# Happy-ZZX/PL-VIWO

Hardware: AMD Instinct MI355X
Metric: frames/sec (track+EKF update), 752x480 mono, 250 pts+80 lines; ATE vs CPU ref (higher is better)
Workload: dtype f64

## Files before the change

pl-viwo_amd/csrc/jacobian_api.hip:

```cpp
#include <algorithm>
#include <vector>

#include <chrono>
#include "jacobian_kernels.hpp"
#include "nullspace_core.hpp"
#include "update_kernels.hpp"
#include "update_state.hpp"
#include "camera_tracks.hpp"

using namespace plv;

#define TRY(expr)                  \
  do {                             \
    int _rc = (expr);              \
    if (_rc != PLV_OK) return _rc; \
  } while (0)

namespace {

int check_views(const plv_state_view *st, const plv_tracks *tr) {
  if (!st || !tr || st->n_clones < 1 || !st->clone_time || !st->clone_R || !st->clone_p || !st->clone_R_fej ||
      !st->clone_p_fej || !st->clone_state_id || tr->n_feat < 1 || !tr->obs_ptr || !tr->obs_time || !tr->obs_uv ||
      !tr->p_FinG || !tr->p_FinG_fej) {
    set_last_error("jacobians: null view field");
// ... 380 lines not shown
  us->pt_tri_p = (const double *)(us->tri.as<char>() + ft.o_p), us->pt_tri_ok = (const unsigned char *)(us->tri.as<char>() + ft.o_ok), us->pt_tri_F = F;
  const bool mirrored = ctx->mirror2_taken;
  ctx->mirror2_src = nullptr, ctx->mirror2_dst = nullptr, ctx->mirror2_bytes = 0, ctx->mirror2_taken = false;
  if (!mirrored)
    PLV_HIP_CHECK(plv::memcpy_async(us->h_tri.p, us->tri.as<char>() + ft.o_p, mirror_bytes, hipMemcpyDeviceToHost, ctx->stream));
  ph_b.stop();
  plv::frame_mark("@ point chain enqueued");
  if (J.chain_events) (void)hipEventRecord(g_ce[2], ctx->stream);
  J.pending = true, J.mirrored = mirrored, J.rc = rc, J.F = F, J.spec = spec != nullptr, J.max_sel = max_sel;
  J.o_p = ft.o_p, J.o_member = ft.o_member, J.o_words = ft.o_words;
  return PLV_OK;
}

int plv_points_update_collect(plv_ctx *ctx, double *p_out, uint8_t *ok_out, double *err_out, uint8_t *accepted, int *n_rows, double *dx,
                              void (*before_wait)(void *), void *before_wait_arg, uint8_t *member, int *spec_count, int *spec_over) {
  if (!ctx || !p_out || !ok_out || !err_out || !accepted || !dx) return PLV_E_BADARG;
  auto *us = plv_update_state(ctx);
  PointJob &J = point_job(ctx);
  if (!J.pending) {
    set_last_error("plv_points_update_collect: no point update was submitted");
    return PLV_E_BADARG;
  }
  J.pending = false;
  int rc = J.rc;
  const int F = J.F;
  plv::HostPhase ph_c("points fused: host work inside the wait");
  if (before_wait) before_wait(before_wait_arg);
  if (rc == PLV_OK && ctx->wait_poll && us->done_ev) {
    while (hipEventQuery(us->done_ev) == hipErrorNotReady || plv::knob(plv::PLV_KNOB_CHAIN_ALWAYS)) {
      if (ctx->wait_poll(ctx->wait_poll_arg)) break;
      for (int i = 0; i < 32; ++i) __builtin_ia32_pause();
    }
  }
  ph_c.stop();
  plv::frame_mark("@ host work inside the point wait done");
  plv::NsScope ns_pw(plv::counters().points_wait_ns);
  plv::HostPhase ph_d("points fused: wait");
  if (J.spec && us->spec_save_seq) spec_save_arm(ctx, us, true);
  if (rc == PLV_OK) rc = plv_msckf_update_resident_wait(ctx, accepted, n_rows, dx);
  spec_save_arm(ctx, us, false);
  if (rc != PLV_OK || !J.mirrored) PLV_HIP_CHECK(plv::stream_sync(ctx->stream));
  ph_d.stop();
  plv::frame_mark("@ point update collected");
  if (J.chain_events) {
    const double host_us = std::chrono::duration<double, std::micro>(std::chrono::steady_clock::now() - J.t_entry).count();
    (void)hipEventSynchronize(g_ce[2]);
    float a = 0.f, b = 0.f;
    if (hipEventElapsedTime(&a, g_ce[0], g_ce[1]) == hipSuccess && hipEventElapsedTime(&b, g_ce[1], g_ce[2]) == hipSuccess) {
      plv::host_phases().add("points fused: DEVICE entry -> Jacobian launch done", a * 1e3);
      plv::host_phases().add("points fused: DEVICE Jacobian done -> last kernel done", b * 1e3);
      plv::host_phases().add("points fused: HOST entry -> results read", host_us);
    }
  }
  const char *h = us->h_tri.as<char>();
  memcpy(p_out, h, (size_t)F * 24);
  memcpy(err_out, h + (size_t)F * 24, (size_t)F * 8);
  memcpy(ok_out, h + (size_t)F * 32, (size_t)F);
  if (J.spec) {
    if (member) memcpy(member, h + (J.o_member - J.o_p), (size_t)F);
    const int *w = (const int *)(h + (J.o_words - J.o_p));
    if (spec_count) *spec_count = w[0];
    if (spec_over) *spec_over = w[1] ? 1 : ((w[3] && w[4] >= J.max_sel) ? 2 : 0);
  } else {
    if (spec_count) *spec_count = 0;
    if (spec_over) *spec_over = 0;
  }
// ... 587 lines not shown
```

pl-viwo_amd/csrc/line_api.hip:

```cpp
#include <algorithm>
#include <chrono>
#include <cmath>
#include <cstring>
#include <atomic>
#include <condition_variable>
#include <functional>
#include <memory>
#include <map>
#include <mutex>
#include <thread>
#include <unordered_map>
#include <vector>

#include "line_host.hpp"
#include "cam_models.hpp"
#include "line_kernels.hpp"
#include "update_state.hpp"
#include "plv_internal.hpp"
#include "camera_tracks.hpp"

using namespace plv;
using namespace plv::linehost;

int plv_tracker_last(plv_ctx *ctx, float *pts, uint64_t *ids, int cap, int *n);
// ... 65 lines not shown
  int early_w = 0, early_h = 0;
  int pending_which = -1, pending_fed = -1;
  bool defer_finish = false;
  std::function<void()> deferred;
  std::atomic<int> defer_state{0};
  struct TriState {
    bool valid = false;
    plv_state_view view;
    std::vector<double> clone_time, clone_R, clone_p;
    std::vector<int> clone_id;
  } tri_state;
  std::vector<float> cached;
  int cached_which = -1, cached_fed = -1;
  std::mutex mtx;
  linehost::Job job;
  std::thread worker;
  std::mutex jm;
  std::condition_variable jcv;
  std::atomic<int> job_state{0};
  struct FeedJob {
    plv_ctx *ctx = nullptr;
    double timestamp = 0, vps[6] = {0, 0, 0, 0, 0, 0};
    double K8[8] = {0, 0, 0, 0, 0, 0, 0, 0};
    int cam_model = 0;
    std::vector<float> pts;
    std::vector<uint64_t> pids;
    int rc = PLV_OK;
    bool pool_on = false;
    PoolArgs pool_args;
  } feed;
  std::atomic<int> feed_state{0};
  std::chrono::steady_clock::time_point job_posted, feed_posted;
  linehost::HostStage host;
};

std::mutex g_mtx;
std::unordered_map<plv_ctx *, LineTracker *> g_lt;
LineTracker *ltr(plv_ctx *ctx, bool run_deferred = true);


void form_line_pool(LineTracker *T, const PoolArgs &A, LinePool &R);
void discard_line_pool(LineTracker *T);
int (*g_feed_impl)(plv_ctx *, LineTracker *, double, const double *, int, const float *, const uint64_t *, const double *, int) = nullptr;
void line_worker(LineTracker *T) {
  for (;;) {
    bool do_detect = false, do_feed = false, do_deferred = false;
    {
      std::unique_lock<std::mutex> lk(T->jm);
      wait_polling(lk, T->jcv, [&] { return T->job_state == 1 || T->job_state == -1 || T->feed_state == 1 || T->defer_state == 1; });
      if (T->job_state == -1) return;
      do_deferred = T->defer_state == 1;
      do_detect = !do_deferred && T->job_state == 1;
      do_feed = !do_deferred && !do_detect && T->feed_state == 1;
    }
    if (do_deferred) {
      std::function<void()> f;
      f.swap(T->deferred);
      if (f) f();
      {
        std::lock_guard<std::mutex> lk(T->jm);
        T->defer_state = 2;
      }
      T->jcv.notify_all();
      continue;
    }
    if (do_feed) {
      LineTracker::FeedJob &F = T->feed;
      if (plv::host_phases().on)
        plv::host_phases().add("line worker: feed job starts after its post", std::chrono::duration<double, std::micro>(std::chrono::steady_clock::now() - T->feed_posted).count());
      const auto Fs = std::chrono::steady_clock::now();
      plv::counters().w_feed_start_ns += (unsigned long long)std::chrono::duration_cast<std::chrono::nanoseconds>(Fs - T->feed_posted).count();
      const int rc = g_feed_impl(F.ctx, T, F.timestamp, F.vps, (int)F.pids.size(), F.pts.data(), F.pids.data(), F.K8, F.cam_model);
      if (rc == PLV_OK && F.pool_on) {
        discard_line_pool(T);
        form_line_pool(T, F.pool_args, T->pool_prep);
      }
      F.pool_on = false;
      plv::frame_mark("@ (worker) line feed + pool done");
      plv::counters().w_feed_ns += (unsigned long long)std::chrono::duration_cast<std::chrono::nanoseconds>(std::chrono::steady_clock::now() - Fs).count();
      {
        std::lock_guard<std::mutex> lk(T->jm);
        F.rc = rc;
        T->feed_state = 2;
      }
      T->jcv.notify_all();
      continue;
    }
    const bool timing = plv::knob(plv::PLV_KNOB_LINE_TIMING);
    auto W0 = std::chrono::steady_clock::now();
    (void)hipSetDevice(T->job.device);
    int rc = PLV_OK;
    if (plv::event_sync(T->edges_ready) != hipSuccess) rc = PLV_E_DEVICE;
    if (rc == PLV_OK && T->job.hlab && plv::event_sync(T->labels_ready) != hipSuccess) rc = PLV_E_DEVICE;
    auto W1 = std::chrono::steady_clock::now();
    if (rc == PLV_OK) rc = host_extract(&T->host, T->job, timing);
    {
      auto ns = [](auto a, auto b) { return (unsigned long long)std::chrono::duration_cast<std::chrono::nanoseconds>(b - a).count(); };
      plv::counters().w_wake_ns += ns(T->job_posted, W0);
      plv::counters().w_maps_ns += ns(W0, W1);
      plv::counters().w_extract_ns += ns(W1, std::chrono::steady_clock::now());
    }
    if (plv::host_phases().on)
      plv::host_phases().add("line worker: detect job, post to done", std::chrono::duration<double, std::micro>(std::chrono::steady_clock::now() - T->job_posted).count());
    plv::frame_mark("@ (worker) line detection done");
    if (timing) {
      auto W2 = std::chrono::steady_clock::now();
      auto us = [](auto a, auto b) { return std::chrono::duration<double, std::micro>(b - a).count(); };
      fprintf(stderr, "line worker: woke %.1f us after the post, edge maps %.1f us, walk + fit %.1f us\n", us(T->job_posted, W0), us(W0, W1), us(W1, W2));
    }
    {
      std::lock_guard<std::mutex> lk(T->jm);
      T->job.rc = rc;
      if (T->job_state == 1) T->job_state = 2;
    }
    T->jcv.notify_all();
  }
}
// ... 815 lines not shown
  bool any = false;
  for (int l = 0; l < Lp; ++l) any = (J.flags[l] = J.valid_n[l] >= 2) || any;
  if (!any) {
    J.stage = LinesJob::FUSED_NOTHING;
    return PLV_OK;
  }
  plv::HostPhase ph_cols("update_lines: columns");
  int rc = plv_line_jacobian_columns(st, &all, J.cols.data(), (int)J.cols.size(), &J.k);
  ph_cols.stop();
  if (rc == PLV_OK && J.k > 0) {
    plv::HostPhase ph_sub("update_lines: fused submit (gate prepare + stage + upload + launch)");
    ctx->gate_rows_hint = 2 * J.most_valid;
    ch.on = chained;
    rc = plv_lines_update_fused_submit(ctx, st, st_tri, &all, J.flags.data(), cap, J.k, J.cols.data(), 2 * opt->max_obs, st->sigma_pix * st->sigma_pix,
                                       opt->chi2_mult);
    ch.on = false;
    if (rc == PLV_OK) {
      J.stage = LinesJob::FUSED_LAUNCHED;
      return PLV_OK;
    }
  }
  if (rc == PLV_OK) {
    J.stage = LinesJob::FUSED_NOTHING;
    return PLV_OK;
  }
  J.stage = LinesJob::FAILED, J.rc = rc;
  return PLV_OK;
}

}
namespace plv {
int plv_camera_lines_submit_chained(plv_ctx *ctx, const plv_state_view *st, const plv_update_options *opt, int cap) {
  if (!ctx || !st || !opt || opt->cpi || st->n_clones < 2 || opt->max_obs < 2 || st->dt_state_id >= 0 || !ctx->chain.ready) return 0;
  LineTracker *T = ltr(ctx);
  if (T->ujob.pending || T->feed.rc != PLV_OK) return 0;
  plv::frame_mark("@ chained first half starts");
  plv::HostPhase ph("update_lines: first half inside the point update's wait (chained)");
  T->tri_state.valid = false;
  (void)lines_first_half(ctx, T, st, st, opt, cap, T->ujob, true);
  if (T->ujob.stage == LinesJob::TWO_STEP) {
    T->pool_prep = std::move(T->ujob.LP);
    T->pool_prep.valid = true;
    T->ujob = LinesJob();
    return 0;
  }
  T->ujob.pending = true;
  plv::frame_mark("@ chained first half done (line launch enqueued)");
  if (T->ujob.stage == LinesJob::FUSED_LAUNCHED) ++plv::counters().chained;
  return 1;
}

int plv_camera_lines_job_pending(plv_ctx *ctx) { return ltr(ctx, false)->ujob.pending ? 1 : 0; }
void plv_camera_lines_job_abort2(plv_ctx *ctx, int keep_pool) {
  LineTracker *T = ltr(ctx, false);
  if (!T->ujob.pending) return;
  (void)plv::stream_sync(ctx->stream);
  ctx->gate_stage.on = 0, ctx->gate_stage_taken = false;
  T->pool_prep = std::move(T->ujob.LP);
  T->pool_prep.valid = true;
  if (!keep_pool) discard_line_pool(T);
  T->ujob = LinesJob();
}
void plv_camera_lines_job_abort(plv_ctx *ctx) { plv_camera_lines_job_abort2(ctx, 0); }
}
extern "C" {

int plv_camera_update_lines(plv_ctx *ctx, const plv_state_view *st, const plv_update_options *opt, double *dx,
                            plv_update_result *res, uint64_t *line_ids, uint8_t *accepted_out, double *lines_out, int cap) {
  if (!ctx || !st || !opt || !dx || !res || st->n_clones < 2 || opt->max_obs < 2) return PLV_E_BADARG;
  LineTracker *T = ltr(ctx);
  *res = plv_update_result{0, 0, 0, 0, 0, PLV_OK, 0, 0, 0};
  const bool timing = plv::knob(plv::PLV_KNOB_UPDATE_TIMING);
  plv::NsScope ns_lines(plv::counters().lines_ns);
  plv::HostPhase ph_all("update_lines: whole call");
  plv::RoctxRange rx_line("[Time-Cam] LINE update");
  auto since = [&](std::chrono::steady_clock::time_point a) { return std::chrono::duration<double, std::micro>(std::chrono::steady_clock::now() - a).count(); };
  LinesJob Jlocal;
  const bool resumed = T->ujob.pending && T->ujob.cap == cap && T->ujob.n_clones == st->n_clones && T->ujob.state_time == opt->state_time &&
                       T->ujob.t_prev_frame == opt->t_prev_frame;
  if (T->ujob.pending && !resumed) {
    plv::set_last_error("plv_camera_update_lines: a chained submission for another window is pending");
    return PLV_E_BADARG;
// ... 231 lines not shown
```

pl-viwo_amd/csrc/plv_ctx.hpp:

```cpp
#pragma once
#include <hip/hip_runtime.h>
#include <sys/resource.h>

#include "gate_stage.hpp"
#include <cstdint>
#include <cstdio>
#include <execinfo.h>
#include <cstring>
#include <algorithm>
#include <atomic>
#include <chrono>
#include <cstdlib>
#include <mutex>
#include <string>
#include <unordered_map>
#include <vector>

#include "../../include/plviwo.h"

namespace plv {

void set_last_error(const char *fmt, ...);

#define PLV_HIP_CHECK(expr)                                                              \
// ... 408 lines not shown
    bool ready = false, on = false;
    std::vector<double> q;
    std::vector<int> ids;
    double qe[4] = {0, 0, 0, 1};
    std::vector<int> anc_ptr, anc_f;
    std::vector<unsigned char> anc_has_old;
    std::vector<double> anc_old;
  } chain;
  int *applied_word = nullptr;
  bool applied_used = false;
  const int *cap_words = nullptr;
  int cap = 0;
  double *cov_save = nullptr;
  unsigned *cov_save_word = nullptr;
  unsigned cov_save_seq = 0;
  const int *skip_word = nullptr;
  const void *mirror2_src = nullptr;
  void *mirror2_dst = nullptr;
  size_t mirror2_bytes = 0;
  bool mirror2_taken = false;
  bool probe = false, probe_done = false;
  const void *probe_src = nullptr;
  void *probe_dst = nullptr;
  int probe_stride_a = 0, probe_off_b = 0, probe_stride_b = 0;
  void (*probe_hook)(void *) = nullptr;
  void *probe_hook_arg = nullptr;

  plv::GateStage gate_stage{};
  bool gate_stage_taken = false;
  int gate_rows_hint = 0;

  int (*wait_poll)(void *) = nullptr;
  void *wait_poll_arg = nullptr;

  void *fe_state = nullptr;
};
```

pl-viwo_amd/csrc/plv_internal.hpp:

```cpp
#pragma once
#include <cstdint>

#include "../../include/plviwo.h"

struct plv_ctx_update_state;

struct plv_points_spec {
  int n_flow;
  const int *li;
  const uint8_t *meta, *prevalid;
  const float *d_flow_p1, *d_flow_n1;
  const uint8_t *d_flow_mask;
};

namespace plv {

plv_ctx_update_state *plv_update_state(plv_ctx *ctx);
int plv_update_gate_prepare(plv_ctx *ctx, int F, int fdim, int k, int ld, double sigma2, double chi2_mult, double res_norm_gate, int probe);
int plv_prior_prefetch(plv_ctx *ctx, int phase, const int *d_cols, int k, int F, int mp_max);

int plv_state_vars_check(int n_var, const plv_state_var *vars, int n_dx);

void plv_frontend_destroy(plv_ctx *ctx);
int plv_feed_image_enqueue(plv_ctx *ctx, const uint8_t *img, int stride);
int plv_front_fed_count(plv_ctx *ctx);
int plv_front_match_device(plv_ctx *ctx, const float **d_p1, const float **d_n1, const uint8_t **d_mask, int *n);
const uint8_t *plv_front_level0(plv_ctx *ctx, int which, int *w, int *h);
int plv_front_quiesce(plv_ctx *ctx);
int plv_perform_detection_ahead(plv_ctx *ctx, const uint8_t *mask, const float *pts, const uint64_t *ids, int n_in);

void plv_tracker_destroy(plv_ctx *ctx);
int plv_point_chain_lookup(plv_ctx *ctx, uint64_t id);
int plv_point_used_lookup(plv_ctx *ctx, uint64_t id, double *p);
void plv_point_anchor_fill(plv_ctx *ctx, int Lp, const int *pt_ptr, const int *pt_ids, int chained, double *anchor, uint8_t *has);
void plv_point_used_cleanup(plv_ctx *ctx, double t_oldest);
void plv_tracker_run_deferred(void *ctx);

void plv_line_tracker_destroy(plv_ctx *ctx);
int plv_line_prefetch_enabled(plv_ctx *ctx);
void plv_line_edges_early(plv_ctx *ctx, const uint8_t *d_raw, int W, int H, const unsigned *d_hist);
int plv_line_tracker_feed_async_points(plv_ctx *ctx, double timestamp, const double *vps, int np, const float *pts, const uint64_t *pids);
void plv_line_defer_finish(plv_ctx *ctx, int on);
void plv_line_run_deferred(plv_ctx *ctx);
int plv_line_pool_prepare(plv_ctx *ctx, const plv_state_view *st, const plv_update_options *opt);
void plv_line_feed_pool_args(plv_ctx *ctx, const plv_state_view *st, const plv_update_options *opt);
void plv_line_pool_discard(plv_ctx *ctx);
int plv_line_db_size_after_feed(plv_ctx *ctx);
int plv_camera_lines_submit_chained(plv_ctx *ctx, const plv_state_view *st, const plv_update_options *opt, int cap);
int plv_camera_lines_job_pending(plv_ctx *ctx);
void plv_camera_lines_job_abort2(plv_ctx *ctx, int keep_pool);
void plv_camera_lines_job_abort(plv_ctx *ctx);

int plv_points_update_submit(plv_ctx *ctx, const plv_state_view *st, const plv_tracks *all, const plv_tri_options *tri,
                             const uint8_t *flags, int max_sel, int k, const int *col_to_state, int ld, double sigma2,
                             double chi2_mult, double res_norm_gate, const plv_points_spec *spec);
int plv_points_update_collect(plv_ctx *ctx, double *p_out, uint8_t *ok_out, double *err_out, uint8_t *accepted, int *n_rows, double *dx,
                              void (*before_wait)(void *), void *before_wait_arg, uint8_t *member, int *spec_count, int *spec_over);
int plv_points_spec_undo(plv_ctx *ctx);
int plv_points_update_fused(plv_ctx *ctx, const plv_state_view *st, const plv_tracks *all, const plv_tri_options *tri,
                            const uint8_t *flags, int max_sel, int k, const int *col_to_state, int ld, double sigma2,
                            double chi2_mult, double res_norm_gate, double *p_out, uint8_t *ok_out, double *err_out,
                            uint8_t *accepted, int *n_rows, double *dx, void (*before_wait)(void *), void *before_wait_arg);
int plv_lines_update_fused(plv_ctx *ctx, const plv_state_view *st, const plv_state_view *st_tri, const plv_line_tracks *all,
                           const uint8_t *flags, int max_sel, int k, const int *col_to_state, int ld, double sigma2,
                           double chi2_mult, double *lines_out, uint8_t *ok_out, uint8_t *accepted, int *n_rows, double *dx,
                           void (*before_wait)(void *), void *before_wait_arg);
int plv_lines_update_fused_submit(plv_ctx *ctx, const plv_state_view *st, const plv_state_view *st_tri, const plv_line_tracks *all,
                                  const uint8_t *flags, int max_sel, int k, const int *col_to_state, int ld, double sigma2, double chi2_mult);
int plv_lines_update_fused_finish(plv_ctx *ctx, double sigma2, double chi2_mult, double *lines_out, uint8_t *ok_out, uint8_t *accepted,
                                  int *n_rows, double *dx, void (*before_wait)(void *), void *before_wait_arg);

}
// ... 1 lines not shown
```

pl-viwo_amd/csrc/tracker_api.hip:

```cpp
#include <algorithm>
#include <functional>
#include <memory>
#include <mutex>
#include <unordered_map>
#include <vector>

#include <sys/resource.h>
#include "plv_ctx.hpp"
#include "update_state.hpp"
#include "plv_internal.hpp"
#include "gate_stage.hpp"
#include "camera_tracks.hpp"

using plv::Track;

namespace {

struct Tracker {
  std::vector<float> pts_last;
  std::vector<uint64_t> ids_last;
  std::vector<uint8_t> mask_last;
  uint64_t currid = 0;
  int detect_ahead = 2;
  bool ahead_deferred = false;
  bool defer_db = false;
  const plv_state_view *early_st = nullptr;
  const plv_update_options *early_lines = nullptr;
  int early_cap = 0;
  std::unordered_map<uint64_t, int> chain_index;
  bool chain_ok = false;
  std::function<void()> deferred_db;
  std::unordered_map<uint64_t, Track> db;
  struct UsedPoint {
    double p[3], newest;
  };
  std::unordered_map<uint64_t, UsedPoint> used;
  struct Listed {
    uint64_t id;
    Track tr;
    double p[3];
  };
  std::vector<Listed> last_slam, last_init;
  std::vector<uint64_t> dec_ids;
  std::vector<double> dec_vals;
  const plv_state_view *spec_st = nullptr;
  const plv_update_options *spec_opt = nullptr;
  std::function<void(int, const float *, const uint64_t *)> points_ready;
  unsigned long long feed_seq = 0;
  std::vector<double> frame_t;
  struct Spec {
    bool active = false;
    double t_prev_frame = 0, state_time = 0, dt = 0, t_oldest = 0, t_oldest2 = 0;
    int n_clones = 0, max_msckf = 0, max_obs = 0, k = 0, F = 0;
    std::unordered_map<uint64_t, int> index;
    std::vector<uint64_t> ids;
    std::vector<int> ptr, li, cols;
    std::vector<uint8_t> meta, prevalid, flags;
    std::vector<double> ot;
    std::vector<float> ouv, ouvn;
  } spec;
  std::mutex mtx;
};

std::mutex g_mtx;
std::unordered_map<plv_ctx *, Tracker *> g_trk;
Tracker *trk(plv_ctx *ctx) {
  std::lock_guard<std::mutex> lk(g_mtx);
  auto it = g_trk.find(ctx);
  if (it != g_trk.end()) return it->second;
// ... 331 lines not shown
    Track &tr = tp[i] ? *tp[i] : T->db[ids[i]];
    if (tr.t.capacity() == 0) {
      tr.t.reserve(32);
      tr.uv.reserve(64);
      tr.uvn.reserve(64);
    }
    tr.t.push_back(timestamp);
    tr.uv.push_back(x);
    tr.uv.push_back(y);
    tr.uvn.push_back(n1[2 * i]);
    tr.uvn.push_back(n1[2 * i + 1]);
  }
  T->pts_last.swap(good);
  T->ids_last.swap(good_ids);
  keep_mask();
  T->ahead_deferred = T->detect_ahead == 2 && !T->ids_last.empty();
  if (T->detect_ahead == 1 && !T->ids_last.empty())
    (void)plv_perform_detection_ahead(ctx, mask, T->pts_last.data(), T->ids_last.data(), (int)T->ids_last.size());
  return PLV_OK;
}

static void start_detection_ahead(void *arg) {
  plv_ctx *ctx = (plv_ctx *)arg;
  Tracker *T = trk(ctx);
  {
    std::lock_guard<std::mutex> lk(T->mtx);
    if (T->ahead_deferred) {
      T->ahead_deferred = false;
      (void)plv_perform_detection_ahead(ctx, T->mask_last.empty() ? nullptr : T->mask_last.data(), T->pts_last.data(), T->ids_last.data(),
                                        (int)T->ids_last.size());
    }
  }
}
static int poll_line_pool(void *arg) {
  plv_ctx *ctx = (plv_ctx *)arg;
  Tracker *T = trk(ctx);
  if (!T->early_lines || !T->early_st) return 1;
  if (!plv_line_pool_prepare(ctx, T->early_st, T->early_lines)) return 0;
  if (plv::host_phases().on) {
    plv::host_phases().add("chain: pool ready inside the point wait (count)", 1.0);
    if (!T->chain_ok) plv::host_phases().add("chain: no - the point pool exceeds max_msckf or holds no candidate (count)", 1.0);
    if (!ctx->chain.ready) plv::host_phases().add("chain: no - state variables not chainable (count)", 1.0);
    if (!plv_update_state(ctx)->applied_armed) plv::host_phases().add("chain: no - the point launch did not arm the applied word (count)", 1.0);
  }
  if (T->chain_ok && ctx->chain.ready && plv_update_state(ctx)->applied_armed && !plv::knob(plv::PLV_KNOB_NO_CHAIN))
    (void)plv_camera_lines_submit_chained(ctx, T->early_st, T->early_lines, T->early_cap);
  return 1;
}
}
namespace plv {
int plv_point_chain_lookup(plv_ctx *ctx, uint64_t id) {
  Tracker *T = trk(ctx);
  auto it = T->chain_index.find(id);
  return it == T->chain_index.end() ? -1 : it->second;
}
}
extern "C" {

int plv_decision_trace(plv_ctx *ctx, int on) {
  if (!ctx) return PLV_E_BADARG;
  ctx->decision_trace = on != 0;
  return PLV_OK;
}
int plv_last_point_decisions(plv_ctx *ctx, uint64_t *ids, double *vals, int cap, int *n) {
  if (!ctx || !n || cap < 0 || (cap > 0 && (!ids || !vals))) return PLV_E_BADARG;
  Tracker *T = trk(ctx);
  *n = (int)T->dec_ids.size();
  if (*n > cap) return cap == 0 ? PLV_OK : PLV_E_CAPACITY;
  std::copy(T->dec_ids.begin(), T->dec_ids.end(), ids);
  std::copy(T->dec_vals.begin(), T->dec_vals.end(), vals);
  return PLV_OK;
}

int plv_tracker_detect_ahead(plv_ctx *ctx, int on) {
  if (!ctx) return PLV_E_BADARG;
  Tracker *T = trk(ctx);
  std::lock_guard<std::mutex> lk(T->mtx);
  T->detect_ahead = on < 0 ? 0 : on > 2 ? 2 : on;
  return PLV_OK;
}
// ... 261 lines not shown
    if (!spec_done) std::fill(dx, dx + ctx->cov_n, 0.0);
    return finish(PLV_OK);
  }
  std::vector<double> pf(3 * (size_t)Fp), err(Fp);
  std::vector<uint8_t> ok(Fp);
  plv_tracks all{};
  all.n_feat = Fp;
  all.obs_ptr = ptr.data();
  all.obs_time = ot.data();
  all.obs_uv = ouv.data();
  all.obs_uvn = ouvn.data();
  if (cpi.on) {
    all.res_R = cpi.R.data();
    all.res_p = cpi.p.data();
  }
  std::vector<int> cols(ctx->cfg.max_state_dim > 0 ? ctx->cfg.max_state_dim : 1024);
  int k = 0, n_rows = 0, rc = PLV_OK;
  const bool fused = !opt->cpi && opt->max_slam == 0 && most_valid <= opt->max_obs;
  ph_pool.stop();
  rx_get.stop();
  plv::frame_mark("@ update_points: pool + staging done");
  plv::RoctxRange rx_upd("[Time-Cam] MSCKF update");
  plv::HostPhase ph_dev("update_points: device submission + wait");
  std::vector<uint8_t> acc_all(Fp, 0);
  bool fused_ran = false;
  if (fused && spec_done) {
    std::copy(s_pf.begin(), s_pf.end(), pf.begin());
    std::copy(s_err.begin(), s_err.end(), err.begin());
    std::copy(s_ok.begin(), s_ok.end(), ok.begin());
    std::copy(s_acc.begin(), s_acc.end(), acc_all.begin());
    n_rows = s_rows;
    res->status = s_status;
    fused_ran = true;
  } else if (fused) {
    std::vector<uint8_t> flags(Fp);
    bool any = false;
    for (int f = 0; f < Fp; ++f) any = (flags[f] = valid_n[f] >= 2) || any;
    if (any) {
      all.p_FinG = all.p_FinG_fej = pf.data();
      rc = plv_jacobian_columns(st, &all, cols.data(), (int)cols.size(), &k);
      if (rc == PLV_OK && k > 0) {
        ctx->gate_rows_hint = 2 * most_valid;
        T->chain_index.clear();
        T->chain_ok = Fp <= opt->max_msckf;
        if (T->chain_ok && T->early_lines)
          for (int f = 0; f < Fp; ++f)
            if (flags[f]) T->chain_index.emplace(pool[f].id, f);
        plv::frame_mark("@ update_points: columns done, fused call");
        rc = plv_points_update_fused(ctx, st, &all, &opt->tri, flags.data(), opt->max_msckf, k, cols.data(), 2 * opt->max_obs,
                                     st->sigma_pix * st->sigma_pix, opt->chi2_mult, 3.0, pf.data(), ok.data(), err.data(), acc_all.data(),
                                     &n_rows, dx, start_detection_ahead, ctx);
        T->chain_ok = false;
        res->status = rc == PLV_E_NOT_PSD ? rc : PLV_OK;
        if (rc == PLV_E_NOT_PSD) {
          rc = PLV_OK;
          std::fill(dx, dx + ctx->cov_n, 0.0);
        }
        fused_ran = rc == PLV_OK;
      }
      if (rc != PLV_OK) {
        for (Cand &c : pool) give_back_all(unused, c);
        return finish(rc);
      }
    }
  } else {
    start_detection_ahead(ctx);
    rc = plv_triangulate(ctx, st, &all, &opt->tri, pf.data(), ok.data(), err.data());
    if (rc != PLV_OK) {
      for (Cand &c : pool) give_back_all(unused, c);
      return finish(rc);
    }
  }
  ph_dev.stop();
  rx_upd.stop();
  if (ctx->decision_trace) {
    const double nan = std::numeric_limits<double>::quiet_NaN();
    T->dec_ids.resize(Fp);
    T->dec_vals.assign((size_t)Fp * PLV_DECISION_VALUES, nan);
    std::vector<double> tri(4 * (size_t)Fp, nan), gate(3 * (size_t)Fp, nan);
    if (fused_ran && ctx->dec_F == Fp) {
      PLV_HIP_CHECK(hipMemcpy(tri.data(), ctx->d_tri_dbg.p, tri.size() * 8, hipMemcpyDeviceToHost));
      if (ctx->dec_gate) PLV_HIP_CHECK(hipMemcpy(gate.data(), ctx->d_gate_dec.p, gate.size() * 8, hipMemcpyDeviceToHost));
    }
    ctx->dec_F = 0, ctx->dec_gate = false;
    for (int f = 0; f < Fp; ++f) {
      double *v = &T->dec_vals[(size_t)f * PLV_DECISION_VALUES];
      T->dec_ids[f] = pool[f].id;
      v[0] = valid_n[f], v[1] = ok[f], v[2] = ok[f] ? err[f] : nan, v[3] = fused_ran ? acc_all[f] : nan;
      for (int i = 0; i < 4; ++i) v[4 + i] = tri[4 * (size_t)f + i];
      for (int i = 0; i < 3; ++i) v[8 + i] = gate[3 * (size_t)f + i];
    }
  }
  plv::RoctxRange rx_db("[Time-Cam] DB clan up");
  plv::HostPhase ph_post("update_points: selection + database");
  std::vector<int> sel;
  std::vector<int> n_skip(Fp, 0);
  for (int f = 0; f < Fp; ++f) {
    Cand &c = pool[f];
    if ((int)sel.size() >= opt->max_msckf) {
      give_back_all(unused, c);
      continue;
    }
    const int valid = valid_n[f];
    if (valid >= 2 && ok[f]) {
      std::lock_guard<std::mutex> lk(T->mtx);
      Tracker::UsedPoint &u = T->used[c.id];
      std::copy(pf.begin() + 3 * (size_t)f, pf.begin() + 3 * (size_t)f + 3, u.p);
      u.newest = c.tr.t.back();
    }
    if (valid < 2 || !ok[f] || !(err[f] < 3.0)) {
      give_back_all(unused, c);
      continue;
    }
    if (valid >= opt->init_min_meas && opt->n_slam + (int)T->last_init.size() < opt->max_slam) {
      Tracker::Listed e{c.id, Track{}, {pf[3 * (size_t)f], pf[3 * (size_t)f + 1], pf[3 * (size_t)f + 2]}};
      for (size_t i = 0; i < c.tr.t.size(); ++i) {
        if (start_of(c.tr.t[i] + dt) < 0)
          give_back(unused, c.id, c.tr, i);
        else
          append_obs(e.tr, c.tr, i);
      }
      T->last_init.push_back(std::move(e));
      continue;
    }
    if (valid > opt->max_obs) {
      n_skip[f] = valid - opt->max_obs;
      ++res->n_truncated;
    }
    sel.push_back(f);
  }
  res->n_msckf = (int)sel.size();
  res->n_init = (int)T->last_init.size();
  if (plv::host_phases().on && Fp > opt->max_msckf) fprintf(stderr, "[plv over] pool %d selected %d\n", Fp, (int)sel.size());
  if (sel.empty()) {
    if (!fused_ran) std::fill(dx, dx + ctx->cov_n, 0.0);
    return finish(PLV_OK);
  }
  const int F = (int)sel.size();
// ... 102 lines not shown
  Tracker *T = trk(ctx);
  std::lock_guard<std::mutex> lk(T->mtx);
  Tracker::UsedPoint &u = T->used[id];
  std::copy(p_FinG, p_FinG + 3, u.p);
  u.newest = newest_obs_time;
  return PLV_OK;
}

}
namespace plv {
int plv_point_used_lookup(plv_ctx *ctx, uint64_t id, double *p) {
  Tracker *T = trk(ctx);
  std::lock_guard<std::mutex> lk(T->mtx);
  auto it = T->used.find(id);
  if (it == T->used.end()) return 0;
  std::copy(it->second.p, it->second.p + 3, p);
  return 1;
}
void plv_point_anchor_fill(plv_ctx *ctx, int Lp, const int *pt_ptr, const int *pt_ids, int chained, double *anchor, uint8_t *has) {
  Tracker *T = trk(ctx);
  std::lock_guard<std::mutex> lk(T->mtx);
  plv_ctx::ChainState &ch = ctx->chain;
  if (chained) ch.anc_ptr.assign(1, 0), ch.anc_f.clear(), ch.anc_has_old.clear(), ch.anc_old.clear();
  for (int l = 0; l < Lp; ++l) {
    uint64_t seen[16];
    int n_seen = 0;
    for (int q = pt_ptr[l]; q < pt_ptr[l + 1]; ++q) {
      const uint64_t id = (uint64_t)pt_ids[q];
      bool dup = false;
      for (int z = 0; z < n_seen && !dup; ++z) dup = seen[z] == id;
      if (dup) continue;
      if (n_seen < 16) seen[n_seen++] = id;
      const auto it = T->used.find(id);
      const bool has_old = it != T->used.end();
      if (!chained) {
        if (!has_old) continue;
        std::copy(it->second.p, it->second.p + 3, anchor + 3 * (size_t)l);
        has[l] = 1;
        break;
      }
      const auto ci = T->chain_index.find(id);
      const int pf = ci == T->chain_index.end() ? -1 : ci->second;
      if (pf < 0 && !has_old) continue;
      static const double zero[3] = {0, 0, 0};
      const double *old = has_old ? it->second.p : zero;
      ch.anc_f.push_back(pf);
      ch.anc_has_old.push_back(has_old ? 1 : 0);
      ch.anc_old.insert(ch.anc_old.end(), old, old + 3);
      if (has_old) break;
    }
    if (chained) ch.anc_ptr.push_back((int)ch.anc_f.size());
  }
}
void plv_point_used_cleanup(plv_ctx *ctx, double t_oldest) {
  Tracker *T = trk(ctx);
  std::lock_guard<std::mutex> lk(T->mtx);
  for (auto it = T->used.begin(); it != T->used.end();)
    it = it->second.newest < t_oldest ? T->used.erase(it) : std::next(it);
}

void plv_tracker_run_deferred(void *arg) {
  plv_ctx *ctx = (plv_ctx *)arg;
  Tracker *T = trk(ctx);
  if (!T->deferred_db) return;
  std::function<void()> f;
  f.swap(T->deferred_db);
  f();
}
}
extern "C" {

static int try_update_args(plv_ctx *ctx, const plv_state_view *st, const plv_try_update *io) {
  if (!ctx || !st || !io || !io->opt_points || !io->dx_points || !io->res_points || (io->n_var > 0 && !io->vars)) return PLV_E_BADARG;
  if (io->opt_lines && (!io->dx_lines || !io->res_lines)) return PLV_E_BADARG;
  if (io->opt_points->max_slam > 0) {
    plv::set_last_error("plv_camera_try_update: max_slam > 0 needs the two-call form (plv_slam_update in between)");
    return PLV_E_BADARG;
  }
// ... 18 lines not shown
  T->early_st = io->opt_lines ? st : nullptr;
  T->early_lines = io->opt_lines;
  T->early_cap = io->line_cap;
  T->chain_ok = false;
  plv_ctx::ChainState &ch = ctx->chain;
  ch.ready = false;
  if (io->opt_lines && io->n_var > 0 && st->dt_state_id < 0 && !io->opt_lines->cpi) {
    const int N = st->n_clones;
    auto find = [&](int kind, int id, int size) -> const plv_state_var * {
      for (int i = 0; i < io->n_var; ++i)
        if (io->vars[i].kind == kind && io->vars[i].id == id && (kind == PLV_VAR_QUAT || io->vars[i].size == size)) return &io->vars[i];
      return nullptr;
    };
    bool okc = true;
    ch.q.assign(4 * (size_t)N, 0.0), ch.ids.assign(N + 3, -1);
    for (int i = 0; i < N && okc; ++i) {
      const int sid = st->clone_state_id[i];
      const plv_state_var *vq = find(PLV_VAR_QUAT, sid, 3), *vp = find(PLV_VAR_VEC, sid + 3, 3);
      const double *vR = st->clone_R + 9 * (size_t)i, *vP = st->clone_p + 3 * (size_t)i;
      okc = sid >= 0 && vq && vp && (vq->out == vR || vq->mirror == vR) && (vp->val == vP || vp->mirror == vP);
      if (okc) std::copy(vq->val, vq->val + 4, ch.q.begin() + 4 * (size_t)i), ch.ids[i] = sid;
    }
    if (okc && st->extrinsic_state_id >= 0) {
      const plv_state_var *vq = find(PLV_VAR_QUAT, st->extrinsic_state_id, 3), *vp = find(PLV_VAR_VEC, st->extrinsic_state_id + 3, 3);
      okc = vq && vp;
      if (okc) std::copy(vq->val, vq->val + 4, ch.qe), ch.ids[N] = st->extrinsic_state_id;
    }
    if (okc && st->intrinsic_state_id >= 0) {
      okc = find(PLV_VAR_VEC, st->intrinsic_state_id, 8) != nullptr;
      ch.ids[N + 1] = st->intrinsic_state_id;
    }
    ch.ready = okc;
  }
  plv::frame_mark("@ try_update: chain state ready");
  ctx->wait_poll = io->opt_lines ? poll_line_pool : nullptr;
  ctx->wait_poll_arg = ctx;
  int rc = plv_camera_update_points(ctx, st, io->opt_points, io->dx_points, io->res_points, io->msckf_ids, io->msckf_accepted, io->p_FinG);
  ctx->wait_poll = nullptr;
  ch.ready = false;
  T->defer_db = false;
  T->early_st = nullptr, T->early_lines = nullptr;
  bool chained = io->opt_lines && plv_camera_lines_job_pending(ctx);
  if (chained && (plv_update_state(ctx)->last_route >= 5 || io->res_points->status != PLV_OK)) {
    if (plv_update_state(ctx)->last_route >= 5) ++plv::counters().route[6];
    plv_camera_lines_job_abort2(ctx, rc == PLV_OK ? 1 : 0);
    chained = false;
  }
  const int rc_lf = rc == PLV_OK && io->opt_lines && !chained ? plv_camera_get_line_features(ctx, st) : PLV_OK;
  plv::frame_mark("@ update_points returned");
  if (rc == PLV_OK) rc = apply(*io->res_points, io->dx_points);
  if (rc == PLV_OK) rc = rc_lf;
  if (rc == PLV_OK && io->opt_lines) {
    rc = plv_line_tracker_feed_wait(ctx);
    io->line_db_size = plv_line_db_size_after_feed(ctx);
    if (rc == PLV_OK) {
      plv_line_defer_finish(ctx, 1);
      rc = plv_camera_update_lines(ctx, st, io->opt_lines, io->dx_lines, io->res_lines, io->line_ids, io->line_accepted, io->line_FinG,
                                   io->line_cap);
      plv_line_defer_finish(ctx, 0);
      plv::frame_mark("@ update_lines returned");
    }
    plv_tracker_run_deferred(ctx);
    if (rc == PLV_OK) rc = apply(*io->res_lines, io->dx_lines);
    plv::frame_mark("@ line dx applied");
  }
  if (rc != PLV_OK && io->opt_lines) {
    if (plv_camera_lines_job_pending(ctx)) plv_camera_lines_job_abort(ctx);
    plv_line_pool_discard(ctx);
  }
  plv_tracker_run_deferred(ctx);
  return rc;
}

int plv_camera_frame(plv_ctx *ctx, const plv_state_view *st, plv_camera_frame_io *io) {
  if (!ctx || !st || !io || (io->slot < 0 && !io->img)) return PLV_E_BADARG;
  const int rc_args = io->update ? try_update_args(ctx, st, io->update) : PLV_OK;
  plv_try_update *const upd = rc_args == PLV_OK ? io->update : nullptr;
  plv::NsScope ns(plv::counters().frame_ns);
  struct RuScope {
    struct rusage a;
    bool on = plv::host_phases().on;
    RuScope() {
      if (on) getrusage(RUSAGE_THREAD, &a);
    }
    ~RuScope() {
      if (!on) return;
      struct rusage b;
      getrusage(RUSAGE_THREAD, &b);
      plv::host_phases().add("frame: minor page faults of the caller's thread (count)", (double)(b.ru_minflt - a.ru_minflt));
      plv::host_phases().add("frame: system time of the caller's thread", (double)((b.ru_stime.tv_sec - a.ru_stime.tv_sec) * 1000000L + (b.ru_stime.tv_usec - a.ru_stime.tv_usec)));
      plv::host_phases().add("frame: involuntary context switches (count)", (double)(b.ru_nivcsw - a.ru_nivcsw));
      plv::host_phases().add("frame: voluntary context switches (count)", (double)(b.ru_nvcsw - a.ru_nvcsw));
    }
  } ru_scope;
  if (plv::host_phases().on)
    plv::frame_t0_ns().store(std::chrono::duration_cast<std::chrono::nanoseconds>(std::chrono::steady_clock::now().time_since_epoch()).count());
  plv::RoctxRange rx_feed("[Time-Cam] feed measurement");
  Tracker *Tf = trk(ctx);
  struct SpecGuard {
    plv_ctx *c;
    Tracker *T;
    ~SpecGuard() {
// ... 56 lines not shown
```

Baseline: 2198.

## Hand chained line-update first half to the line worker after its feed

Lets the point-update wait loop (or the caller after collecting the point update) offer the chained line-update first half to the line worker thread, which runs it immediately after finishing the line feed instead of the main thread waiting for the feed. A snapshot of the clone state and a 'used before' map of point anchors are kept so the worker sees consistent pre-update anchors. This removes serialization between the line feed completion and the line first-half launch, at the cost of extra cross-thread handshakes, state copying and more complex chain bookkeeping.

```diff
diff --git a/pl-viwo_amd/csrc/jacobian_api.hip b/pl-viwo_amd/csrc/jacobian_api.hip
--- a/pl-viwo_amd/csrc/jacobian_api.hip
+++ b/pl-viwo_amd/csrc/jacobian_api.hip
@@ -436,6 +436,7 @@
       for (int i = 0; i < 32; ++i) __builtin_ia32_pause();
     }
   }
+  if (ctx->wait_poll_end) ctx->wait_poll_end(ctx->wait_poll_arg);
   ph_c.stop();
   plv::frame_mark("@ host work inside the point wait done");
   plv::NsScope ns_pw(plv::counters().points_wait_ns);
diff --git a/pl-viwo_amd/csrc/line_api.hip b/pl-viwo_amd/csrc/line_api.hip
--- a/pl-viwo_amd/csrc/line_api.hip
+++ b/pl-viwo_amd/csrc/line_api.hip
@@ -121,6 +121,10 @@
   std::atomic<int> feed_state{0};
   std::chrono::steady_clock::time_point job_posted, feed_posted;
   linehost::HostStage host;
+  std::atomic<int> chain_claim{0};
+  const plv_state_view *chain_st = nullptr;
+  const plv_update_options *chain_opt = nullptr;
+  int chain_cap = 0;
 };
 
 std::mutex g_mtx;
@@ -130,6 +134,7 @@
 
 void form_line_pool(LineTracker *T, const PoolArgs &A, LinePool &R);
 void discard_line_pool(LineTracker *T);
+int chained_first_half(plv_ctx *ctx, LineTracker *T, const plv_state_view *st, const plv_update_options *opt, int cap);
 int (*g_feed_impl)(plv_ctx *, LineTracker *, double, const double *, int, const float *, const uint64_t *, const double *, int) = nullptr;
 void line_worker(LineTracker *T) {
   for (;;) {
@@ -166,12 +171,23 @@
       }
       F.pool_on = false;
       plv::frame_mark("@ (worker) line feed + pool done");
-      plv::counters().w_feed_ns += (unsigned long long)std::chrono::duration_cast<std::chrono::nanoseconds>(std::chrono::steady_clock::now() - Fs).count();
+      bool stage = false;
       {
         std::lock_guard<std::mutex> lk(T->jm);
         F.rc = rc;
+        stage = T->chain_claim == 1;
+        if (stage) T->chain_claim = 2;
+        else T->feed_state = 2;
+      }
+      if (stage) {
+        (void)hipSetDevice(F.ctx->device);
+        const int staged = chained_first_half(F.ctx, T, T->chain_st, T->chain_opt, T->chain_cap);
+        if (plv::host_phases().on) plv::host_phases().add(staged ? "chain: staged by the line worker at the end of its feed (count)" : "chain: no - the line worker's staging declined (count)", 1.0);
+        std::lock_guard<std::mutex> lk(T->jm);
+        T->chain_claim = 3;
         T->feed_state = 2;
       }
+      plv::counters().w_feed_ns += (unsigned long long)std::chrono::duration_cast<std::chrono::nanoseconds>(std::chrono::steady_clock::now() - Fs).count();
       T->jcv.notify_all();
       continue;
     }
@@ -1053,7 +1069,12 @@
 namespace plv {
 int plv_camera_lines_submit_chained(plv_ctx *ctx, const plv_state_view *st, const plv_update_options *opt, int cap) {
   if (!ctx || !st || !opt || opt->cpi || st->n_clones < 2 || opt->max_obs < 2 || st->dt_state_id >= 0 || !ctx->chain.ready) return 0;
-  LineTracker *T = ltr(ctx);
+  return chained_first_half(ctx, ltr(ctx), st, opt, cap);
+}
+}
+namespace {
+int chained_first_half(plv_ctx *ctx, LineTracker *T, const plv_state_view *st, const plv_update_options *opt, int cap) {
+  if (!ctx || !st || !opt || opt->cpi || st->n_clones < 2 || opt->max_obs < 2 || st->dt_state_id >= 0 || !ctx->chain.ready) return 0;
   if (T->ujob.pending || T->feed.rc != PLV_OK) return 0;
   plv::frame_mark("@ chained first half starts");
   plv::HostPhase ph("update_lines: first half inside the point update's wait (chained)");
@@ -1069,6 +1090,36 @@
   plv::frame_mark("@ chained first half done (line launch enqueued)");
   if (T->ujob.stage == LinesJob::FUSED_LAUNCHED) ++plv::counters().chained;
   return 1;
+}
+LineTracker *ltr_peek(plv_ctx *ctx) {
+  std::lock_guard<std::mutex> lk(g_mtx);
+  auto it = g_lt.find(ctx);
+  return it == g_lt.end() ? nullptr : it->second;
+}
+}
+namespace plv {
+int plv_line_chain_offer(plv_ctx *ctx, const plv_state_view *st, const plv_update_options *opt, int cap) {
+  LineTracker *T = ltr_peek(ctx);
+  if (!T) return 0;
+  std::lock_guard<std::mutex> lk(T->jm);
+  if (T->feed_state != 1 || T->chain_claim != 0) return 0;
+  T->chain_st = st, T->chain_opt = opt, T->chain_cap = cap;
+  T->chain_claim = 1;
+  return 1;
+}
+int plv_line_chain_taken(plv_ctx *ctx) {
+  LineTracker *T = ltr_peek(ctx);
+  return T && T->chain_claim == 3 ? 1 : 0;
+}
+int plv_line_chain_close(plv_ctx *ctx) {
+  LineTracker *T = ltr_peek(ctx);
+  if (!T) return 0;
+  std::unique_lock<std::mutex> lk(T->jm);
+  if (T->chain_claim == 2) wait_polling(lk, T->jcv, [&] { return T->chain_claim == 3; });
+  const int staged = T->chain_claim == 3 ? 1 : 0;
+  T->chain_claim = 0;
+  T->chain_st = nullptr, T->chain_opt = nullptr;
+  return staged;
 }
 
 int plv_camera_lines_job_pending(plv_ctx *ctx) { return ltr(ctx, false)->ujob.pending ? 1 : 0; }
diff --git a/pl-viwo_amd/csrc/plv_ctx.hpp b/pl-viwo_amd/csrc/plv_ctx.hpp
--- a/pl-viwo_amd/csrc/plv_ctx.hpp
+++ b/pl-viwo_amd/csrc/plv_ctx.hpp
@@ -464,6 +464,7 @@
 
   int (*wait_poll)(void *) = nullptr;
   void *wait_poll_arg = nullptr;
+  void (*wait_poll_end)(void *) = nullptr;
 
   void *fe_state = nullptr;
 };
diff --git a/pl-viwo_amd/csrc/plv_internal.hpp b/pl-viwo_amd/csrc/plv_internal.hpp
--- a/pl-viwo_amd/csrc/plv_internal.hpp
+++ b/pl-viwo_amd/csrc/plv_internal.hpp
@@ -38,6 +38,9 @@
 
 void plv_line_tracker_destroy(plv_ctx *ctx);
 int plv_line_prefetch_enabled(plv_ctx *ctx);
+int plv_line_chain_offer(plv_ctx *ctx, const plv_state_view *st, const plv_update_options *opt, int cap);
+int plv_line_chain_taken(plv_ctx *ctx);
+int plv_line_chain_close(plv_ctx *ctx);
 void plv_line_edges_early(plv_ctx *ctx, const uint8_t *d_raw, int W, int H, const unsigned *d_hist);
 int plv_line_tracker_feed_async_points(plv_ctx *ctx, double timestamp, const double *vps, int np, const float *pts, const uint64_t *pids);
 void plv_line_defer_finish(plv_ctx *ctx, int on);
diff --git a/pl-viwo_amd/csrc/tracker_api.hip b/pl-viwo_amd/csrc/tracker_api.hip
--- a/pl-viwo_amd/csrc/tracker_api.hip
+++ b/pl-viwo_amd/csrc/tracker_api.hip
@@ -29,12 +29,31 @@
   int early_cap = 0;
   std::unordered_map<uint64_t, int> chain_index;
   bool chain_ok = false;
+  bool chain_polled = false;
+  bool chain_armed = false;
+  bool chain_handed = false;
+  bool chain_staged = false;
+  struct StateCopy {
+    plv_state_view view{};
+    std::vector<double> t, R, p, Rf, pf;
+    std::vector<int> id;
+    void take(const plv_state_view *st) {
+      const size_t N = (size_t)std::max(st->n_clones, 0);
+      view = *st;
+      auto copy = [](auto &v, const auto *src, size_t n) { return src ? (v.assign(src, src + n), v.data()) : nullptr; };
+      view.clone_time = copy(t, st->clone_time, N), view.clone_R = copy(R, st->clone_R, 9 * N), view.clone_p = copy(p, st->clone_p, 3 * N);
+      view.clone_R_fej = copy(Rf, st->clone_R_fej, 9 * N), view.clone_p_fej = copy(pf, st->clone_p_fej, 3 * N);
+      view.clone_state_id = copy(id, st->clone_state_id, N);
+    }
+  } early_copy;
   std::function<void()> deferred_db;
   std::unordered_map<uint64_t, Track> db;
   struct UsedPoint {
     double p[3], newest;
   };
   std::unordered_map<uint64_t, UsedPoint> used;
+  bool keep_used_before = false;
+  std::unordered_map<uint64_t, std::pair<bool, UsedPoint>> used_before;
   struct Listed {
     uint64_t id;
     Track tr;
@@ -432,10 +451,23 @@
     }
   }
 }
+static void arm_chain(plv_ctx *ctx, Tracker *T) {
+  if (T->chain_polled) return;
+  T->chain_polled = true;
+  T->chain_armed = T->chain_ok && ctx->chain.ready && plv_update_state(ctx)->applied_armed && !plv::knob(plv::PLV_KNOB_NO_CHAIN);
+}
 static int poll_line_pool(void *arg) {
   plv_ctx *ctx = (plv_ctx *)arg;
   Tracker *T = trk(ctx);
   if (!T->early_lines || !T->early_st) return 1;
+  if (T->chain_handed) return plv_line_chain_taken(ctx);
+  if (!T->chain_polled) {
+    arm_chain(ctx, T);
+    if (T->chain_armed && plv_line_chain_offer(ctx, &T->early_copy.view, T->early_lines, T->early_cap)) {
+      T->chain_handed = true;
+      return 0;
+    }
+  }
   if (!plv_line_pool_prepare(ctx, T->early_st, T->early_lines)) return 0;
   if (plv::host_phases().on) {
     plv::host_phases().add("chain: pool ready inside the point wait (count)", 1.0);
@@ -443,9 +475,40 @@
     if (!ctx->chain.ready) plv::host_phases().add("chain: no - state variables not chainable (count)", 1.0);
     if (!plv_update_state(ctx)->applied_armed) plv::host_phases().add("chain: no - the point launch did not arm the applied word (count)", 1.0);
   }
-  if (T->chain_ok && ctx->chain.ready && plv_update_state(ctx)->applied_armed && !plv::knob(plv::PLV_KNOB_NO_CHAIN))
+  if (T->chain_armed) {
+    T->chain_staged = true;
     (void)plv_camera_lines_submit_chained(ctx, T->early_st, T->early_lines, T->early_cap);
+  }
   return 1;
+}
+static void end_line_poll(void *arg) {
+  plv_ctx *ctx = (plv_ctx *)arg;
+  Tracker *T = trk(ctx);
+  if (T->early_lines && T->early_st) arm_chain(ctx, T);
+  if (!T->chain_handed) return;
+  T->chain_handed = false;
+  if (plv_line_chain_close(ctx)) T->chain_staged = true;
+}
+static void chain_after_collect(plv_ctx *ctx, Tracker *T, int status) {
+  if (!T->chain_armed || T->chain_staged || T->chain_handed || !T->early_lines || !T->early_st) return;
+  if (status != PLV_OK || plv_update_state(ctx)->last_route >= 5) return;
+  T->chain_staged = true;
+  if (!ctx->decision_trace) {
+    {
+      std::lock_guard<std::mutex> lk(T->mtx);
+      T->keep_used_before = true;
+    }
+    if (plv_line_chain_offer(ctx, &T->early_copy.view, T->early_lines, T->early_cap)) {
+      T->chain_handed = true;
+      if (plv::host_phases().on) plv::host_phases().add("chain: offered to the line worker after the point update was collected (count)", 1.0);
+      return;
+    }
+    std::lock_guard<std::mutex> lk(T->mtx);
+    T->keep_used_before = false;
+  }
+  if (!plv_line_pool_prepare(ctx, T->early_st, T->early_lines)) return;
+  if (plv::host_phases().on) plv::host_phases().add("chain: staged by the caller after the point update was collected (count)", 1.0);
+  (void)plv_camera_lines_submit_chained(ctx, T->early_st, T->early_lines, T->early_cap);
 }
 }
 namespace plv {
@@ -773,6 +836,7 @@
     n_rows = s_rows;
     res->status = s_status;
     fused_ran = true;
+    chain_after_collect(ctx, T, s_status);
   } else if (fused) {
     std::vector<uint8_t> flags(Fp);
     bool any = false;
@@ -784,6 +848,7 @@
         ctx->gate_rows_hint = 2 * most_valid;
         T->chain_index.clear();
         T->chain_ok = Fp <= opt->max_msckf;
+        T->chain_polled = T->chain_armed = false;
         if (T->chain_ok && T->early_lines)
           for (int f = 0; f < Fp; ++f)
             if (flags[f]) T->chain_index.emplace(pool[f].id, f);
@@ -793,6 +858,7 @@
                                      &n_rows, dx, start_detection_ahead, ctx);
         T->chain_ok = false;
         res->status = rc == PLV_E_NOT_PSD ? rc : PLV_OK;
+        if (rc == PLV_OK) chain_after_collect(ctx, T, PLV_OK);
         if (rc == PLV_E_NOT_PSD) {
           rc = PLV_OK;
           std::fill(dx, dx + ctx->cov_n, 0.0);
@@ -845,6 +911,10 @@
     const int valid = valid_n[f];
     if (valid >= 2 && ok[f]) {
       std::lock_guard<std::mutex> lk(T->mtx);
+      if (T->keep_used_before) {
+        const auto it = T->used.find(c.id);
+        T->used_before.emplace(c.id, it == T->used.end() ? std::make_pair(false, Tracker::UsedPoint{}) : std::make_pair(true, it->second));
+      }
       Tracker::UsedPoint &u = T->used[c.id];
       std::copy(pf.begin() + 3 * (size_t)f, pf.begin() + 3 * (size_t)f + 3, u.p);
       u.newest = c.tr.t.back();
@@ -1013,7 +1083,7 @@
       if (dup) continue;
       if (n_seen < 16) seen[n_seen++] = id;
       const auto it = T->used.find(id);
-      const bool has_old = it != T->used.end();
+      bool has_old = it != T->used.end();
       if (!chained) {
         if (!has_old) continue;
         std::copy(it->second.p, it->second.p + 3, anchor + 3 * (size_t)l);
@@ -1022,9 +1092,13 @@
       }
       const auto ci = T->chain_index.find(id);
       const int pf = ci == T->chain_index.end() ? -1 : ci->second;
-      if (pf < 0 && !has_old) continue;
       static const double zero[3] = {0, 0, 0};
       const double *old = has_old ? it->second.p : zero;
+      if (T->keep_used_before) {
+        const auto b = T->used_before.find(id);
+        if (b != T->used_before.end()) has_old = b->second.first, old = has_old ? b->second.second.p : zero;
+      }
+      if (pf < 0 && !has_old) continue;
       ch.anc_f.push_back(pf);
       ch.anc_has_old.push_back(has_old ? 1 : 0);
       ch.anc_old.insert(ch.anc_old.end(), old, old + 3);
@@ -1109,26 +1183,45 @@
     }
     ch.ready = okc;
   }
+  T->chain_polled = T->chain_armed = T->chain_handed = T->chain_staged = false;
+  if (ch.ready) T->early_copy.take(st);
   plv::frame_mark("@ try_update: chain state ready");
   ctx->wait_poll = io->opt_lines ? poll_line_pool : nullptr;
+  ctx->wait_poll_end = io->opt_lines ? end_line_poll : nullptr;
   ctx->wait_poll_arg = ctx;
   int rc = plv_camera_update_points(ctx, st, io->opt_points, io->dx_points, io->res_points, io->msckf_ids, io->msckf_accepted, io->p_FinG);
   ctx->wait_poll = nullptr;
-  ch.ready = false;
+  ctx->wait_poll_end = nullptr;
   T->defer_db = false;
   T->early_st = nullptr, T->early_lines = nullptr;
-  bool chained = io->opt_lines && plv_camera_lines_job_pending(ctx);
+  const bool handed = T->chain_handed;
+  auto settle_chain = [&]() {
+    if (T->chain_handed) {
+      T->chain_handed = false;
+      (void)plv_line_chain_close(ctx);
+      std::lock_guard<std::mutex> lk(T->mtx);
+      T->keep_used_before = false;
+      T->used_before.clear();
+    }
+    ch.ready = false;
+  };
+  if (!handed) ch.ready = false;
+  bool chained = io->opt_lines && !handed && plv_camera_lines_job_pending(ctx);
   if (chained && (plv_update_state(ctx)->last_route >= 5 || io->res_points->status != PLV_OK)) {
     if (plv_update_state(ctx)->last_route >= 5) ++plv::counters().route[6];
     plv_camera_lines_job_abort2(ctx, rc == PLV_OK ? 1 : 0);
     chained = false;
   }
-  const int rc_lf = rc == PLV_OK && io->opt_lines && !chained ? plv_camera_get_line_features(ctx, st) : PLV_OK;
+  const int rc_lf = rc == PLV_OK && io->opt_lines && !chained && !handed ? plv_camera_get_line_features(ctx, st) : PLV_OK;
   plv::frame_mark("@ update_points returned");
   if (rc == PLV_OK) rc = apply(*io->res_points, io->dx_points);
   if (rc == PLV_OK) rc = rc_lf;
   if (rc == PLV_OK && io->opt_lines) {
     rc = plv_line_tracker_feed_wait(ctx);
+    if (handed) {
+      settle_chain();
+      if (rc == PLV_OK && !plv_camera_lines_job_pending(ctx)) rc = plv_camera_get_line_features(ctx, &T->early_copy.view);
+    }
     io->line_db_size = plv_line_db_size_after_feed(ctx);
     if (rc == PLV_OK) {
       plv_line_defer_finish(ctx, 1);
@@ -1142,9 +1235,11 @@
     plv::frame_mark("@ line dx applied");
   }
   if (rc != PLV_OK && io->opt_lines) {
+    settle_chain();
     if (plv_camera_lines_job_pending(ctx)) plv_camera_lines_job_abort(ctx);
     plv_line_pool_discard(ctx);
   }
+  settle_chain();
   plv_tracker_run_deferred(ctx);
   return rc;
 }
```

Measured after the change: 2148 (median of 2 runs). 2.3% lower.
